# RunpeiDong/ACT

Hardware: AMD Instinct MI355X
Metric: stage2_pretrain_point_clouds_per_sec (higher is better)
Workload: dtype f32

## Files before the change

### act_amd/_abi.py

```python
import ctypes

_vp, _i, _f, _sz = ctypes.c_void_p, ctypes.c_int, ctypes.c_float, ctypes.c_size_t
_u, _u64, _ll, _str = ctypes.c_uint, ctypes.c_uint64, ctypes.c_longlong, ctypes.c_char_p
_d = ctypes.c_double
_P = ctypes.POINTER


class GemmEpilogue(ctypes.Structure):
    _fields_ = [("alpha", _f), ("act", _i), ("accumulate", _i), ("rows_per_scale", _i), ("ldr", _i), ("ldaux", _i),
                ("res_row_div", _i), ("bias", _vp), ("rowscale", _vp), ("res", _vp), ("aux", _vp)]


class GemmTnProblem(ctypes.Structure):
    _fields_ = [("A", _vp), ("lda", _i), ("B", _vp), ("ldb", _i), ("C", _vp), ("ldc", _i), ("M", _i), ("N", _i), ("bias_out", _vp)]


class GemmFx(ctypes.Structure):
    _fields_ = ([(n, _vp) for n in ("a_scale", "a_shift", "b_scale", "b_shift", "tile_stats", "gmax", "garg")] + [("group", _i), ("store_c", _i)]
                + [(n, _vp) for n in ("sa_src", "sa_arg", "ep_src", "ep_arg", "row_groups")])


class BlockParams(ctypes.Structure):
    _fields_ = [(n, _vp) for n in ("norm1_w", "norm1_b", "qkv_w", "qkv_b", "proj_w", "proj_b", "norm2_w", "norm2_b",
                                   "fc1_w", "fc1_b", "fc2_w", "fc2_b")]
# ... 92 lines not shown
    "act_bn_tiles_finalize_f32": [_vp, _i, _i, _i, _vp, _vp, _f, _f, _vp, _vp, _vp, _vp, _vp, _vp, _vp],
    "act_layernorm_fwd_f32": [_vp, _vp, _vp, _vp, _vp, _vp, _vp, _vp, _i, _i, _f, _vp],
    "act_prompt_layernorm_fwd_f32": [_vp, _vp, _i, _i, _i, _f, _u64, _vp, _vp, _vp, _f, _vp, _vp],
    "act_prompt_rows_fwd_f32": [_vp, _vp, _vp, _i, _i, _i, _f, _u64, _vp, _vp],
    "act_prompt_rows_bwd_f32": [_vp, _vp, _i, _i, _i, _f, _u64, _vp, _vp, _vp],
    "act_layernorm_bwd_workspace": (_sz, [_i, _i]),
    "act_layernorm_bwd_f32": [_vp, _vp, _vp, _vp, _vp, _vp, _vp, _vp, _vp, _i, _vp, _sz, _i, _i, _vp],
    "act_colsum_workspace": (_sz, [_i, _i]),
    "act_colsum_f32": [_vp, _i, _i, _i, _vp, _i, _vp, _sz, _vp],
    "act_attention_fwd_f32": [_vp, _vp, _vp, _i, _i, _i, _i, _f, _vp],
    "act_attention_fwd_prefix_f32": [_vp, _i, _vp, _i, _vp, _vp, _i, _i, _i, _f, _vp],
    "act_attention_bwd_f32": [_vp, _vp, _vp, _vp, _vp, _i, _i, _i, _i, _f, _vp],
    "act_attention_bwd_prefix_f32": [_vp, _i, _vp, _i, _vp, _vp, _vp, _vp, _vp, _i, _i, _i, _f, _vp],
    "act_cosine_loss_fwd_f32": [_vp, _vp, _i, _i, _f, _vp, _vp, _vp, _vp],
    "act_cosine_loss_bwd_f32": [_vp, _vp, _vp, _vp, _i, _i, _f, _vp, _vp],
    "act_regression_loss_fwd_f32": [_vp, _vp, _i, _i, _i, _vp, _vp, _vp],
    "act_regression_loss_bwd_f32": [_vp, _vp, _vp, _i, _i, _i, _vp, _vp],
    "act_softmax_xent_fwd_f32": [_vp, _vp, _i, _i, _vp, _vp, _vp, _vp],
    "act_softmax_xent_bwd_f32": [_vp, _vp, _vp, _vp, _i, _i, _vp, _vp],
    "act_colstats_workspace": (_sz, [_i, _i]),
    "act_bn_stats_f32": [_vp, _i, _i, _vp, _vp, _f, _f, _vp, _vp, _vp, _vp, _vp, _vp, _vp, _sz, _vp],
    "act_affine_act_f32": [_vp, _vp, _vp, _i, _i, _i, _vp, _vp],
    "act_bn_bwd_f32": [_vp, _vp, _vp, _vp, _vp, _vp, _i, _i, _i, _vp, _vp, _vp, _vp, _sz, _vp],
    "act_bn_bwd_groups_f32": [_vp, _vp, _vp, _vp, _vp, _vp, _i, _i, _i, _vp, _i, _vp, _vp, _vp, _vp, _sz, _vp],
    "act_col_mean_var_f32": [_vp, _i, _i, _vp, _vp, _vp, _sz, _vp],
    "act_bn_bwd_sums_f32": [_vp, _vp, _vp, _vp, _vp, _vp, _i, _i, _i, _vp, _vp, _vp, _sz, _vp],
    "act_bn_bwd_apply_f32": [_vp, _vp, _vp, _vp, _vp, _vp, _vp, _vp, _f, _i, _i, _i, _vp, _vp],
    "act_group_max_f32": [_vp, _i, _i, _i, _vp, _vp, _vp],
    "act_group_max_bwd_f32": [_vp, _vp, _i, _i, _i, _i, _vp, _vp],
    "act_group_max_bwd_matmul_f32": [_vp, _vp, _i, _i, _i, _vp, _i, _i, _vp, _i, _vp],
    "act_group_live_i32": [_vp, _i, _i, _vp, _vp],
    "act_group_max_bwd_matmul_live_f32": [_vp, _vp, _i, _i, _i, _vp, _i, _i, _vp, _i, _vp, _vp],
    "act_group_max_bwd_wgrad_workspace": (_sz, [_i, _i, _i, _i]),
    "act_group_max_bwd_wgrad_f32": [_vp, _vp, _i, _i, _i, _vp, _i, _i, _vp, _vp, _vp, _i, _vp, _sz, _vp],
    "act_group_sum_f32": [_vp, _i, _i, _i, _vp, _vp],
    "act_edge_gn_lrelu_max_f32": [_vp, _i, _i, _vp, _i, _i, _i, _i, _i, _vp, _vp, _f, _f, _vp, _vp, _i, _i, _vp],
    "act_edge_gn_lrelu_max_bwd_f32": [_vp, _i, _i, _vp, _i, _i, _i, _i, _i, _vp, _vp, _vp, _f, _vp, _i, _vp, _vp, _vp, _vp],
    "act_edge_bwd_lds": [_i],
    "act_gn_gumbel_argmax_gather_f32": [_vp, _i, _i, _i, _i, _vp, _vp, _f, _f, _vp, _u64, _vp, _f, _vp, _i, _vp, _vp, _vp, _vp, _vp],
    "act_gumbel_softmax_fwd_f32": [_vp, _i, _i, _vp, _u64, _f, _vp, _vp],
    "act_gumbel_softmax_bwd_f32": [_vp, _vp, _i, _i, _f, _vp, _vp],
    "act_kl_uniform_fwd_f32": [_vp, _i, _i, _i, _vp, _vp, _vp, _vp],
    "act_kl_uniform_bwd_f32": [_vp, _vp, _vp, _vp, _i, _i, _i, _vp, _vp],
    "act_split_bf16x2_f32": [_vp, _i, _i, _i, _vp, _vp, _vp],
    "act_sgemm_nt_bf16x3_supported": [_i, _i, _i],
    "act_sgemm_nt_bf16x3_f32": [_i, _i, _i, _vp, _vp, _vp, _vp, _vp, _i, _epi, _vp],
    "act_layernorm_fwd_planes_f32": [_vp, _vp, _vp, _vp, _vp, _vp, _vp, _vp, _vp, _vp, _i, _i, _f, _vp],
    "act_prompt_layernorm_fwd_planes_f32": [_vp, _vp, _i, _i, _i, _f, _u64, _vp, _vp, _vp, _f, _vp, _vp, _vp],
    "act_attention_fwd_prefix_planes_f32": [_vp, _i, _vp, _i, _vp, _vp, _vp, _vp, _i, _i, _i, _f, _vp],
    "act_sgemm_nt_bf16x3_planes_f32": [_i, _i, _i, _vp, _vp, _vp, _vp, _vp, _i, _vp, _vp, _epi, _vp],
    "act_split_f16x2_f32": [_vp, _i, _i, _i, _f, _vp, _vp, _vp, _vp],
    "act_sgemm_nt_f16x3_supported": [_i, _i, _i],
    "act_sgemm_nt_f16x3_planes_f32": [_i, _i, _i, _vp, _vp, _f, _vp, _vp, _vp, _vp, _i, _vp, _vp, _f, _epi, _vp],
    "act_layernorm_fwd_f16_planes_f32": [_vp, _vp, _vp, _vp, _vp, _vp, _vp, _vp, _f, _vp, _vp, _i, _i, _f, _vp],
    "act_attention_fwd_prefix_f16_planes_f32": [_vp, _i, _vp, _i, _vp, _vp, _vp, _f, _vp, _i, _i, _i, _f, _vp],
    "act_gemm_tune_set": [_i] * 7,
    "act_gemm_tune_get": [_i] * 5 + [_P(_i), _P(_i)],
    "act_gemm_tune_clear": [],
    "act_gemm_tile_info": [_i] + [_P(_i)] * 4,
    "act_scale_rows_f32": [_vp, _vp, _i, _i, _i, _vp, _vp],
    "act_bn_eval_affine_f32": [_vp, _vp, _vp, _vp, _f, _i, _vp, _vp, _vp],
    "act_composite_collect_begin": [],
    "act_composite_collect_end": [_P(_i), _i],
    "act_composite_shutdown": [],
    "act_block_saved_floats": (_sz, [_dims]),
    "act_block_fwd_f32": [_dims, _blk, _vp, _vp, _vp, _vp, _i, _vp, _vp, _vp, _sz, _vp],
    "act_block_bwd_scratch_floats": (_sz, [_dims]),
    "act_block_bwd_f32": [_dims, _blk, _vp, _vp, _vp, _vp, _vp, _blk, _vp, _vp, _sz, _vp, _sz, _vp, _vp],
    "act_block_stack_saved_floats": (_sz, [_dims, _i, _i]),
    "act_block_stack_bwd_scratch_floats": (_sz, [_dims, _i]),
    "act_block_stack_fwd_f32": [_dims, _P(BlockStack), _vp, _vp, _i, _vp, _vp, _vp, _sz, _vp],
    "act_block_stack_bwd_f32": [_dims, _P(BlockStack), _vp, _vp, _vp, _vp, _vp, _vp, _vp, _vp, _sz, _vp, _sz, _vp, _vp],
    "act_add_f32": [_vp, _vp, _vp, _ll, _vp],
    "act_prefix_block_saved_floats": (_sz, [_dims, _i]),
    "act_prefix_block_fwd_f32": [_dims, _i, _blk, _vp, _vp, _vp, _vp, _i, _vp, _vp, _vp, _sz, _vp],
    "act_prefix_block_fwd_kv_f32": [_dims, _i, _blk, _vp, _vp, _vp, _vp, _vp, _vp, _sz, _vp],
    "act_prompt_kv_sparse": [_i],
    "act_prompt_kv_workspace": (_sz, [_i, _i, _i, _i]),
    "act_prompt_kv_fwd_f32": [_vp, _vp, _i, _i, _i, _i, _f, _u64, _vp, _vp, _vp, _f, _vp, _vp, _vp, _vp, _sz, _vp, _sz, _vp],
    "act_prefix_block_bwd_scratch_floats": (_sz, [_dims, _i]),
    "act_prefix_block_bwd_f32": [_dims, _i, _blk, _vp, _vp, _vp, _vp, _vp, _vp, _vp, _sz, _vp],
    "act_prefix_vit_scratch_floats": (_sz, [_P(PrefixVit)]),
    "act_prefix_vit_fwd_bf16x3_f32": [_P(PrefixVit), _x3, _vp, _vp, _vp, _vp, _vp, _sz, _vp],
    "act_prefix_block_fwd_bf16x3_f32": [_dims, _i, _blk, _x3, _vp, _vp, _vp, _i, _vp, _vp, _vp, _sz, _vp],
    "act_prefix_block_bwd_bf16x3_f32": [_dims, _i, _blk, _x3, _vp, _vp, _vp, _vp, _vp, _vp, _vp, _sz, _vp],
    "act_prefix_vit_fwd_f32": [_P(PrefixVit), _vp, _vp, _vp, _vp, _vp, _sz, _vp],
    "act_prefix_vit_fwd_f16x3_f32": [_P(PrefixVit), _P(VitF16x3), _vp, _vp, _vp, _vp, _vp, _sz, _vp],
    "act_pointnet_saved_floats": (_sz, [_pnd]),
    "act_pointnet_fwd_f32": [_pnd, _pnp, _vp, _i, _i, _vp, _vp, _vp, _sz, _vp],
    "act_pointnet_fwd_groups_f32": [_pnd, _pnp, _vp, _i, _i, _vp, _vp, _vp, _i, _vp, _sz, _vp],
    "act_pointnet_bwd_scratch_floats": (_sz, [_pnd]),
    "act_pointnet_bwd_f32": [_pnd, _pnp, _vp, _vp, _vp, _P(PointnetGrads), _vp, _vp, _sz, _vp],
    "act_dgcnn_scratch_floats": (_sz, [_P(Dgcnn)]),
    "act_dgcnn_features_f32": [_P(Dgcnn), _vp, _vp, _vp, _vp, _vp, _sz, _vp],
    "act_dgcnn_features_f16x3_f32": [_P(Dgcnn), _P(DgcnnF16x3), _vp, _vp, _vp, _vp, _vp, _sz, _vp],
    "act_three_nn_f32": [_vp, _vp, _i, _i, _i, _vp, _vp, _vp, _vp, _vp],
    "act_interp_rows_fwd_f32": [_vp, _vp, _vp, _vp, _vp, _vp, _i, _i, _i, _i, _vp, _vp],
    "act_interp_rows_bwd_f32": [_vp, _vp, _vp, _vp, _i, _i, _i, _i, _vp, _vp],
    "act_interp_xyz_grad_workspace": (_sz, [_ll, _i]),
    "act_interp_xyz_grad_f32": [_vp, _vp, _ll, _i, _vp, _vp, _vp, _sz, _vp],
    "act_log_softmax_fwd_f32": [_vp, _ll, _i, _vp, _vp],
    "act_log_softmax_bwd_f32": [_vp, _vp, _ll, _i, _vp, _vp],
    "act_nll_weighted_workspace": (_sz, [_ll]),
    "act_nll_weighted_fwd_f32": [_vp, _vp, _vp, _ll, _i, _vp, _vp, _vp, _vp, _sz, _vp],
    "act_nll_weighted_bwd_f32": [_vp, _vp, _vp, _vp, _ll, _i, _vp, _vp],
    "act_confusion_i64": [_vp, _vp, _ll, _i, _vp, _vp],
# ... 65 lines not shown
```

### act_amd/csrc/gemm_bf16x3.hip

```cpp
#include "gemm_common.h"
#include "split_f16.h"
#include <stdlib.h>

typedef short bf16x8 __attribute__((ext_vector_type(8)));
typedef _Float16 f16x8 __attribute__((ext_vector_type(8)));
typedef unsigned u32x4v __attribute__((ext_vector_type(4)));

namespace {

__device__ __forceinline__ unsigned bf16_rne(float x) {
    unsigned u = __float_as_uint(x);
    u += 0x7FFFu + ((u >> 16) & 1u);
    return u >> 16;
}

__global__ __launch_bounds__(256) void split_bf16x2_kernel(const float* __restrict__ x, int K4, int ldx, long long n4, unsigned short* __restrict__ hi,
                                                           unsigned short* __restrict__ lo) {
    for (long long i = (long long)blockIdx.x * blockDim.x + threadIdx.x; i < n4; i += (long long)gridDim.x * blockDim.x) {
        const long long row = i / K4; const int c4 = (int)(i - row * K4);
        const float4 v = *reinterpret_cast<const float4*>(x + row * ldx + c4 * 4);
        const float e[4] = {v.x, v.y, v.z, v.w};
        unsigned h[4], l[4];
#pragma unroll
        for (int j = 0; j < 4; ++j) {
            h[j] = bf16_rne(e[j]);
            l[j] = bf16_rne(e[j] - __uint_as_float(h[j] << 16));
        }
        reinterpret_cast<uint2*>(hi)[i] = make_uint2(h[0] | (h[1] << 16), h[2] | (h[3] << 16));
        reinterpret_cast<uint2*>(lo)[i] = make_uint2(l[0] | (l[1] << 16), l[2] | (l[3] << 16));
    }
}
__global__ __launch_bounds__(256) void split_f16x2_kernel(const float* __restrict__ x, int K4, int ldx, long long n4, float scale,
                                                          const float* __restrict__ row_scale, unsigned short* __restrict__ h1, unsigned short* __restrict__ h2) {
    for (long long i = (long long)blockIdx.x * blockDim.x + threadIdx.x; i < n4; i += (long long)gridDim.x * blockDim.x) {
        const long long row = i / K4; const int c4 = (int)(i - row * K4);
        const float4 v = *reinterpret_cast<const float4*>(x + row * ldx + c4 * 4);
        store_f16_planes4(h1, h2, (size_t)i, v, row_scale ? scale * row_scale[row] : scale);
    }
}

constexpr int BK = 32;
constexpr int LROW = 40;

struct X3Params {
    const unsigned short *Ah, *Al, *Bh, *Bl;
    float* C; int ldc;
    unsigned short *Oh, *Ol;
    int M, N, K;
    act_gemm_epilogue_t epi;
    const float* b_inv; float a_inv, o_scale;
};

template <bool F16>
__device__ __forceinline__ f32x4 x3_mfma(const bf16x8& b, const bf16x8& a, const f32x4& c) {
    if constexpr (F16) return __builtin_amdgcn_mfma_f32_16x16x32_f16(__builtin_bit_cast(f16x8, b), __builtin_bit_cast(f16x8, a), c, 0, 0, 0);
    else return __builtin_amdgcn_mfma_f32_16x16x32_bf16(b, a, c, 0, 0, 0);
}

template <int BM, int BN, int ACT, bool PLANES, bool F16>
__global__ __launch_bounds__(256, 2) void sgemm_nt_bf16x3_kernel(const X3Params p) {
    constexpr int TM = BM / 32, TN = BN / 32;
    constexpr int PA = BM * LROW, PB = BN * LROW;
    constexpr int NA = BM / 64, NB = BN / 64;
    constexpr int STAGE = 2 * (PA + PB);
    __shared__ __attribute__((aligned(16))) unsigned short L[2 * STAGE];
    const int tid = threadIdx.x, lane = tid & 63, wave = tid >> 6;
    const int wm = wave >> 1, wn = wave & 1;
    const int tiles_n = p.N / BN, tiles_m = p.M / BM;
    int wg = blockIdx.x;
    {
        const int nwg = tiles_m * tiles_n, q = nwg >> 3, r = nwg & 7, xcd = wg & 7, loc = wg >> 3;
        wg = (xcd < r ? xcd * (q + 1) : r * (q + 1) + (xcd - r) * q) + loc;
    }
    constexpr int GM = 8;
    const int per_group = GM * tiles_n, group = wg / per_group, first_m = group * GM;
    const int gsz = min(tiles_m - first_m, GM), in_group = wg - group * per_group;
    const int tile_m = first_m + in_group % gsz, tile_n = in_group / gsz;
    const int m0 = tile_m * BM, n0 = tile_n * BN;
    const int K = p.K, ntiles = K / BK, last = ntiles - 1;

    constexpr int X = F16 ? 1 : 0;
    f32x4 acc[X + 1][TM][TN];
#pragma unroll
    for (int x = 0; x <= X; ++x)
#pragma unroll
        for (int i = 0; i < TM; ++i)
#pragma unroll
            for (int j = 0; j < TN; ++j) acc[x][i][j] = f32x4{0.f, 0.f, 0.f, 0.f};

    const int srow = tid >> 2, sch = tid & 3;
    const size_t goa = (size_t)(m0 + srow) * K + sch * 8, gob = (size_t)(n0 + srow) * K + sch * 8;
    const unsigned short* gA[2] = {p.Ah + goa, p.Al + goa};
    const unsigned short* gB[2] = {p.Bh + gob, p.Bl + gob};
    u32x4v ra0[2][NA], rb0[2][NB], ra1[2][NA], rb1[2][NB];
    const int s_off = srow * LROW + sch * 8;
    const int r = lane & 15, g = lane >> 4;
    const int a_off = (wm * (BM / 2) + r) * LROW + g * 8, b_off = (wn * (BN / 2) + r) * LROW + g * 8;
#define X3_LOAD(RA, RB, T)                                                                                                             \
    _Pragma("unroll") for (int s_ = 0; s_ < 2; ++s_) {                                                                                 \
        _Pragma("unroll") for (int i_ = 0; i_ < NA; ++i_) RA[s_][i_] = *reinterpret_cast<const u32x4v*>(gA[s_] + (size_t)(64 * i_) * K + (T) * BK); \
        _Pragma("unroll") for (int i_ = 0; i_ < NB; ++i_) RB[s_][i_] = *reinterpret_cast<const u32x4v*>(gB[s_] + (size_t)(64 * i_) * K + (T) * BK); \
    }
#define X3_STORE(RA, RB, STG)                                                                                                          \
    _Pragma("unroll") for (int s_ = 0; s_ < 2; ++s_) {                                                                                 \
        _Pragma("unroll") for (int i_ = 0; i_ < NA; ++i_) *reinterpret_cast<u32x4v*>(&L[(STG) * STAGE + s_ * PA + s_off + 64 * i_ * LROW]) = RA[s_][i_];           \
        _Pragma("unroll") for (int i_ = 0; i_ < NB; ++i_) *reinterpret_cast<u32x4v*>(&L[(STG) * STAGE + 2 * PA + s_ * PB + s_off + 64 * i_ * LROW]) = RB[s_][i_];  \
    }
#define X3_COMPUTE(STG)                                                                                                                \
    {                                                                                                                                  \
        const unsigned short* As_ = L + (STG) * STAGE; const unsigned short* Bs_ = As_ + 2 * PA;                                       \
        bf16x8 af[TM][2];                                                                                                              \
        _Pragma("unroll") for (int i_ = 0; i_ < TM; ++i_)                                                                              \
            _Pragma("unroll") for (int s_ = 0; s_ < 2; ++s_) af[i_][s_] = *reinterpret_cast<const bf16x8*>(&As_[s_ * PA + a_off + i_ * 16 * LROW]); \
        _Pragma("unroll") for (int j_ = 0; j_ < TN; ++j_) {                                                                            \
            bf16x8 bf[2];                                                                                                              \
            _Pragma("unroll") for (int s_ = 0; s_ < 2; ++s_) bf[s_] = *reinterpret_cast<const bf16x8*>(&Bs_[s_ * PB + b_off + j_ * 16 * LROW]); \
             \
             \
            _Pragma("unroll") for (int i_ = 0; i_ < TM; ++i_) acc[X][i_][j_] = x3_mfma<F16>(bf[0], af[i_][1], acc[X][i_][j_]);           \
            _Pragma("unroll") for (int i_ = 0; i_ < TM; ++i_) acc[X][i_][j_] = x3_mfma<F16>(bf[1], af[i_][0], acc[X][i_][j_]);           \
            _Pragma("unroll") for (int i_ = 0; i_ < TM; ++i_) acc[0][i_][j_] = x3_mfma<F16>(bf[0], af[i_][0], acc[0][i_][j_]);           \
        }                                                                                                                              \
    }
    X3_LOAD(ra0, rb0, 0)
    X3_LOAD(ra1, rb1, min(1, last))
    X3_STORE(ra0, rb0, 0)
    __syncthreads();
    for (int t = 0; t < ntiles; t += 2) {
        X3_LOAD(ra0, rb0, min(t + 2, last))
        X3_COMPUTE(0)
        X3_STORE(ra1, rb1, 1)
        __syncthreads();
        X3_LOAD(ra1, rb1, min(t + 3, last))
        X3_COMPUTE(1)
        X3_STORE(ra0, rb0, 0)
        __syncthreads();
    }
#undef X3_LOAD
#undef X3_STORE
#undef X3_COMPUTE
    const bool vec = (((uintptr_t)p.C | (uintptr_t)p.epi.bias | (uintptr_t)p.epi.res | (uintptr_t)p.epi.aux) & 15) == 0 &&
                     ((p.ldc | (p.epi.res ? p.epi.ldr : 0) | (p.epi.aux ? p.epi.ldaux : 0)) & 3) == 0;
#pragma unroll
    for (int i = 0; i < TM; ++i)
#pragma unroll
        for (int j = 0; j < TN; ++j) {
            const int row = m0 + wm * (BM / 2) + i * 16 + r;
            const int col = n0 + wn * (BN / 2) + j * 16 + g * 4;
            float4 v = make_float4(acc[0][i][j][0], acc[0][i][j][1], acc[0][i][j][2], acc[0][i][j][3]);
            if constexpr (F16) {
                const float4 bi = *reinterpret_cast<const float4*>(p.b_inv + col);
                constexpr float W = 1.0f / 2048.0f;
                v.x = __builtin_fmaf(acc[1][i][j][0], W, v.x) * bi.x * p.a_inv; v.y = __builtin_fmaf(acc[1][i][j][1], W, v.y) * bi.y * p.a_inv;
                v.z = __builtin_fmaf(acc[1][i][j][2], W, v.z) * bi.z * p.a_inv; v.w = __builtin_fmaf(acc[1][i][j][3], W, v.w) * bi.w * p.a_inv;
            }
            if (vec) v = epilogue_apply4_act<ACT>(p.epi, v, row, col);
            else {
                v.x = epilogue_apply<ACT>(p.epi, v.x, row, col); v.y = epilogue_apply<ACT>(p.epi, v.y, row, col + 1);
                v.z = epilogue_apply<ACT>(p.epi, v.z, row, col + 2); v.w = epilogue_apply<ACT>(p.epi, v.w, row, col + 3);
            }
            if (!PLANES || p.C) {
                float* cp = p.C + (size_t)row * p.ldc + col;
                if (vec) *reinterpret_cast<float4*>(cp) = v; else { cp[0] = v.x; cp[1] = v.y; cp[2] = v.z; cp[3] = v.w; }
            }
            if constexpr (PLANES && F16) {
                store_f16_planes4(p.Oh, p.Ol, ((size_t)row * p.N + col) >> 2, v, p.o_scale);
            } else if constexpr (PLANES) {
                const float e[4] = {v.x, v.y, v.z, v.w};
                unsigned h[4], l[4];
#pragma unroll
                for (int q = 0; q < 4; ++q) { h[q] = bf16_rne(e[q]); l[q] = bf16_rne(e[q] - __uint_as_float(h[q] << 16)); }
                const size_t o = (size_t)row * p.N + col;
                *reinterpret_cast<uint2*>(p.Oh + o) = make_uint2(h[0] | (h[1] << 16), h[2] | (h[3] << 16));
                *reinterpret_cast<uint2*>(p.Ol + o) = make_uint2(l[0] | (l[1] << 16), l[2] | (l[3] << 16));
            }
        }
}

template <int BM, int BN, bool F16>
int launch_x3(const X3Params& p, hipStream_t s) {
    const dim3 grid((p.M / BM) * (p.N / BN));
    const bool planes = p.Oh != nullptr;
    switch (p.epi.act) {
        case ACT_EPI_NONE:
            if (planes) hipLaunchKernelGGL((sgemm_nt_bf16x3_kernel<BM, BN, ACT_EPI_NONE, true, F16>), grid, dim3(256), 0, s, p);
            else        hipLaunchKernelGGL((sgemm_nt_bf16x3_kernel<BM, BN, ACT_EPI_NONE, false, F16>), grid, dim3(256), 0, s, p);
            break;
        case ACT_EPI_GELU:
            if (planes) hipLaunchKernelGGL((sgemm_nt_bf16x3_kernel<BM, BN, ACT_EPI_GELU, true, F16>), grid, dim3(256), 0, s, p);
            else        hipLaunchKernelGGL((sgemm_nt_bf16x3_kernel<BM, BN, ACT_EPI_GELU, false, F16>), grid, dim3(256), 0, s, p);
            break;
        case ACT_EPI_MUL_GELU_GRAD:
            if (planes) hipLaunchKernelGGL((sgemm_nt_bf16x3_kernel<BM, BN, ACT_EPI_MUL_GELU_GRAD, true, F16>), grid, dim3(256), 0, s, p);
            else        hipLaunchKernelGGL((sgemm_nt_bf16x3_kernel<BM, BN, ACT_EPI_MUL_GELU_GRAD, false, F16>), grid, dim3(256), 0, s, p);
            break;
        default: return ACT_E_BADARG;
    }
    ACT_LAUNCH_CHECK();
    return 0;
}

}

extern "C" int act_split_bf16x2_f32(const float* x, int R, int K, int ldx, uint16_t* hi, uint16_t* lo, act_stream_t stream) {
    if (!x || !hi || !lo) return ACT_E_NULLPTR;
    if (R < 0 || K <= 0 || (K & 3) || ldx < K || (ldx & 3) || (((uintptr_t)x | (uintptr_t)hi | (uintptr_t)lo) & 15)) return ACT_E_BADARG;
    const long long n4 = (long long)R * K / 4; if (n4 == 0) return 0;
    hipStream_t s = (hipStream_t)stream;
    ActProfScope ps(KID_ELTWISE, s, 0.0, 8.0 * R * (double)K);
    long long g = (n4 + 255) / 256; if (g > 8192) g = 8192;
    hipLaunchKernelGGL(split_bf16x2_kernel, dim3((unsigned)g), dim3(256), 0, s, x, K / 4, ldx, n4, hi, lo);
    ACT_LAUNCH_CHECK(); return 0;
}

extern "C" int act_sgemm_nt_bf16x3_supported(int M, int N, int K) { return M > 0 && N > 0 && K > 0 && M % 128 == 0 && N % 128 == 0 && K % 64 == 0; }

extern "C" int act_sgemm_nt_bf16x3_f32(int M, int N, int K, const uint16_t* a_hi, const uint16_t* a_lo, const uint16_t* b_hi, const uint16_t* b_lo,
                                       float* C, int ldc, const act_gemm_epilogue_t* epilogue, act_stream_t stream) {
    return act_sgemm_nt_bf16x3_planes_f32(M, N, K, a_hi, a_lo, b_hi, b_lo, C, ldc, nullptr, nullptr, epilogue, stream);
}

extern "C" int act_sgemm_nt_bf16x3_planes_f32(int M, int N, int K, const uint16_t* a_hi, const uint16_t* a_lo, const uint16_t* b_hi, const uint16_t* b_lo,
                                              float* C, int ldc, uint16_t* out_hi, uint16_t* out_lo, const act_gemm_epilogue_t* epilogue,
                                              act_stream_t stream) {
    if (!a_hi || !a_lo || !b_hi || !b_lo || (!C && !out_hi) || ((out_hi == nullptr) != (out_lo == nullptr))) return ACT_E_NULLPTR;
    if (!act_sgemm_nt_bf16x3_supported(M, N, K) || (C && ldc < N)) return ACT_E_BADARG;
    if ((((uintptr_t)a_hi | (uintptr_t)a_lo | (uintptr_t)b_hi | (uintptr_t)b_lo | (uintptr_t)out_hi | (uintptr_t)out_lo) & 15)) return ACT_E_BADARG;
    X3Params p{};
    p.Ah = a_hi; p.Al = a_lo; p.Bh = b_hi; p.Bl = b_lo; p.C = C; p.ldc = ldc; p.M = M; p.N = N; p.K = K; p.Oh = out_hi; p.Ol = out_lo;
    if (epilogue) p.epi = *epilogue; else { p.epi = act_gemm_epilogue_t{}; p.epi.alpha = 1.0f; }
    if (p.epi.accumulate || (p.epi.act != ACT_EPI_NONE && p.epi.act != ACT_EPI_GELU && p.epi.act != ACT_EPI_MUL_GELU_GRAD)) return ACT_E_BADARG;
    hipStream_t s = (hipStream_t)stream;
    ActProfScope ps(KID_GEMM_BF16X3, s, 2.0 * M * (double)N * K, 4.0 * ((double)M * K + (double)N * K + (double)M * N));
    return launch_x3<128, 128, false>(p, s);
}

extern "C" int act_split_f16x2_f32(const float* x, int R, int K, int ldx, float scale, const float* row_scale, uint16_t* h1, uint16_t* h2,
                                   act_stream_t stream) {
    if (!x || !h1 || !h2) return ACT_E_NULLPTR;
    if (R < 0 || K <= 0 || (K & 3) || ldx < K || (ldx & 3) || !(scale > 0.f) || (((uintptr_t)x | (uintptr_t)h1 | (uintptr_t)h2) & 15)) return ACT_E_BADARG;
    const long long n4 = (long long)R * K / 4; if (n4 == 0) return 0;
    hipStream_t s = (hipStream_t)stream;
    ActProfScope ps(KID_ELTWISE, s, 0.0, 8.0 * R * (double)K);
    long long g = (n4 + 255) / 256; if (g > 8192) g = 8192;
    hipLaunchKernelGGL(split_f16x2_kernel, dim3((unsigned)g), dim3(256), 0, s, x, K / 4, ldx, n4, scale, row_scale, h1, h2);
    ACT_LAUNCH_CHECK(); return 0;
}

extern "C" int act_sgemm_nt_f16x3_supported(int M, int N, int K) { return act_sgemm_nt_bf16x3_supported(M, N, K); }

extern "C" int act_sgemm_nt_f16x3_planes_f32(int M, int N, int K, const uint16_t* a_h1, const uint16_t* a_h2, float a_scale, const uint16_t* b_h1,
                                             const uint16_t* b_h2, const float* b_inv_scale, float* C, int ldc, uint16_t* out_h1, uint16_t* out_h2,
                                             float out_scale, const act_gemm_epilogue_t* epilogue, act_stream_t stream) {
    if (!a_h1 || !a_h2 || !b_h1 || !b_h2 || !b_inv_scale || (!C && !out_h1) || ((out_h1 == nullptr) != (out_h2 == nullptr))) return ACT_E_NULLPTR;
    if (!act_sgemm_nt_f16x3_supported(M, N, K) || (C && ldc < N) || !(a_scale > 0.f) || (out_h1 && !(out_scale > 0.f))) return ACT_E_BADARG;
    if ((((uintptr_t)a_h1 | (uintptr_t)a_h2 | (uintptr_t)b_h1 | (uintptr_t)b_h2 | (uintptr_t)out_h1 | (uintptr_t)out_h2 | (uintptr_t)b_inv_scale) & 15))
        return ACT_E_BADARG;
    X3Params p{};
    p.Ah = a_h1; p.Al = a_h2; p.Bh = b_h1; p.Bl = b_h2; p.C = C; p.ldc = ldc; p.M = M; p.N = N; p.K = K; p.Oh = out_h1; p.Ol = out_h2;
    p.b_inv = b_inv_scale; p.a_inv = 1.0f / a_scale; p.o_scale = out_scale;
    if (epilogue) p.epi = *epilogue; else { p.epi = act_gemm_epilogue_t{}; p.epi.alpha = 1.0f; }
    if (p.epi.accumulate || (p.epi.act != ACT_EPI_NONE && p.epi.act != ACT_EPI_GELU && p.epi.act != ACT_EPI_MUL_GELU_GRAD)) return ACT_E_BADARG;
    hipStream_t s = (hipStream_t)stream;
    ActProfScope ps(KID_GEMM_BF16X3, s, 2.0 * M * (double)N * K, 4.0 * ((double)M * K + (double)N * K + (double)M * N));
    return launch_x3<128, 128, true>(p, s);
}
```

### act_amd/kernels.py

```python
import ctypes
import os

import numpy as np

import torch

from . import _C
from ._abi import GemmEpilogue, GemmTnProblem

EPI_NONE, EPI_GELU, EPI_RELU, EPI_MUL_GELU_GRAD, EPI_MUL_RELU_MASK = 0, 1, 2, 3, 4

lib, ptr, stream, check = _C.lib, _C.ptr, _C.stream, _C.check

_WS = {}
_WS_BYTES = 160 << 20


def workspace(device, nbytes=_WS_BYTES, stream_handle=None):
    idx = device.index if device.index is not None else torch.cuda.current_device()
    key = (idx, _C.stream_handle(idx) if stream_handle is None else stream_handle)
    w = _WS.get(key)
    if w is None or w.numel() * 4 < nbytes:
        w = torch.empty(max(nbytes, _WS_BYTES) // 4, dtype=torch.float32, device=device)
        _WS[key] = w
# ... 127 lines not shown
                                           None, None, T, D, float(eps), stream()), "act_layernorm_fwd_planes_f32")
    return planes


def gemm_nt_bf16x3(a_planes, b_planes, bias=None, act=EPI_NONE, res=None, out=None, planes_out=None):
    _, M, Kd = a_planes.shape
    _, N, Kb = b_planes.shape
    if Kd != Kb or a_planes.dtype != torch.bfloat16 or b_planes.dtype != torch.bfloat16 or not (a_planes.is_contiguous() and b_planes.is_contiguous()):
        raise _C.ActHipError("gemm_nt_bf16x3: contiguous bf16 planes [2, rows, K] with equal K expected")
    if not lib.act_sgemm_nt_bf16x3_supported(M, N, Kd):
        raise _C.ActHipError(f"gemm_nt_bf16x3: unsupported shape {M} x {N} x {Kd} (M, N % 128, K % 64)")
    if out is None:
        out = torch.empty(M, N, dtype=torch.float32, device=a_planes.device)
    e = GemmEpilogue(alpha=1.0, act=act, accumulate=0, rows_per_scale=0, ldr=(res.stride(0) if res is not None else 0), ldaux=0, res_row_div=0,
                     bias=ptr(bias), rowscale=None, res=ptr(res), aux=None)
    if planes_out is not None:
        if planes_out.dtype != torch.bfloat16 or tuple(planes_out.shape) != (2, M, N) or not planes_out.is_contiguous():
            raise _C.ActHipError("gemm_nt_bf16x3: planes_out must be a contiguous bf16 tensor [2, M, N]")
        check(lib.act_sgemm_nt_bf16x3_planes_f32(M, N, Kd, ptr(a_planes[0]), ptr(a_planes[1]), ptr(b_planes[0]), ptr(b_planes[1]), ptr(out), out.stride(0),
                                                 ptr(planes_out[0]), ptr(planes_out[1]), ctypes.byref(e), stream()), "act_sgemm_nt_bf16x3_planes_f32")
        return out
    check(lib.act_sgemm_nt_bf16x3_f32(M, N, Kd, ptr(a_planes[0]), ptr(a_planes[1]), ptr(b_planes[0]), ptr(b_planes[1]), ptr(out), out.stride(0),
                                      ctypes.byref(e), stream()), "act_sgemm_nt_bf16x3_f32")
    return out


def f16x3_row_scales(w):
    mx = w.detach().abs().amax(dim=1).float()
    e = torch.frexp(mx).exponent
    e = torch.where(mx > 0, e, torch.full_like(e, 15))
    one = torch.ones(e.shape, dtype=torch.float32, device=w.device)
    return torch.ldexp(one, 15 - e), torch.ldexp(one, e - 15)


def split_f16x2(x, scale=1.0, row_scale=None, out=None):
    x = _f32rows(x, "x")
    R, Kd = x.shape
    if out is None:
        out = torch.empty(2, R, Kd, dtype=torch.float16, device=x.device)
    check(lib.act_split_f16x2_f32(_C.ptr_rows(x), R, Kd, x.stride(0), float(scale), ptr(_f32c(row_scale)) if row_scale is not None else None,
                                  ptr(out[0]), ptr(out[1]), stream()), "act_split_f16x2_f32")
    return out


def layernorm_f16_planes(x, gamma, beta, eps, scale, pos=None):
    x = _f32c(x)
    T, D = x.shape
    planes = torch.empty(2, T, D, dtype=torch.float16, device=x.device)
    check(lib.act_layernorm_fwd_f16_planes_f32(ptr(x), ptr(_f32c(pos)) if pos is not None else None, ptr(gamma), ptr(beta), None, None, ptr(planes[0]),
                                               ptr(planes[1]), float(scale), None, None, T, D, float(eps), stream()), "act_layernorm_fwd_f16_planes_f32")
    return planes


def gemm_nt_f16x3(a_planes, a_scale, b_planes, b_inv_scale, bias=None, act=EPI_NONE, res=None, out=None, planes_out=None, out_scale=1.0):
    _, M, Kd = a_planes.shape
    _, N, Kb = b_planes.shape
    if Kd != Kb or a_planes.dtype != torch.float16 or b_planes.dtype != torch.float16 or not (a_planes.is_contiguous() and b_planes.is_contiguous()):
        raise _C.ActHipError("gemm_nt_f16x3: contiguous f16 planes [2, rows, K] with equal K expected")
    if not lib.act_sgemm_nt_f16x3_supported(M, N, Kd):
        raise _C.ActHipError(f"gemm_nt_f16x3: unsupported shape {M} x {N} x {Kd} (M, N % 128, K % 64)")
    b_inv_scale = _f32c(b_inv_scale)
    if b_inv_scale.numel() != N:
        raise _C.ActHipError("gemm_nt_f16x3: b_inv_scale must hold one value per row of b")
    if out is None:
        out = torch.empty(M, N, dtype=torch.float32, device=a_planes.device)
    e = GemmEpilogue(alpha=1.0, act=act, accumulate=0, rows_per_scale=0, ldr=(res.stride(0) if res is not None else 0), ldaux=0, res_row_div=0,
                     bias=ptr(bias), rowscale=None, res=ptr(res), aux=None)
    oh, ol = (None, None)
    if planes_out is not None:
        if planes_out.dtype != torch.float16 or tuple(planes_out.shape) != (2, M, N) or not planes_out.is_contiguous():
            raise _C.ActHipError("gemm_nt_f16x3: planes_out must be a contiguous f16 tensor [2, M, N]")
        oh, ol = ptr(planes_out[0]), ptr(planes_out[1])
    check(lib.act_sgemm_nt_f16x3_planes_f32(M, N, Kd, ptr(a_planes[0]), ptr(a_planes[1]), float(a_scale), ptr(b_planes[0]), ptr(b_planes[1]), ptr(b_inv_scale),
                                            ptr(out), out.stride(0), oh, ol, float(out_scale), ctypes.byref(e), stream()), "act_sgemm_nt_f16x3_planes_f32")
    return out


_GEMM_CACHE = {}
AUTOTUNE = os.environ.get("ACT_GEMM_AUTOTUNE", "1") != "0"
AUTOTUNE_FULL = os.environ.get("ACT_GEMM_AUTOTUNE", "1") == "full"
_TUNE_FILE = os.environ.get("ACT_GEMM_TUNE_FILE") or os.path.join(os.path.dirname(os.path.abspath(__file__)), "gemm_tune_gfx950.json")
_GEMM_TABLE = {}
_MAX_SPLIT = int(os.environ.get("ACT_GEMM_MAX_SPLIT", "0"))
if os.environ.get("ACT_GEMM_TUNE_TABLE", "1") != "0" and os.path.exists(_TUNE_FILE):
    import json as _json
    with open(_TUNE_FILE) as _fh:
        _GEMM_TABLE = {tuple(int(v) for v in k.split(",")): tuple(c) for k, c in _json.load(_fh)["configs"].items()}
    if _MAX_SPLIT > 0:
        _GEMM_TABLE = {k: c for k, c in _GEMM_TABLE.items() if c[1] <= _MAX_SPLIT or k[4] > 8192}
_NEW_TUNED = {}
if os.environ.get("ACT_GEMM_TUNE_SAVE"):
    import atexit as _atexit

    def _dump_tuned(path=os.environ["ACT_GEMM_TUNE_SAVE"].replace("%p", str(os.getpid()))):
        import json
        merged = dict(_GEMM_TABLE); merged.update(_NEW_TUNED)
        with open(path, "w") as f:
            json.dump({"arch": "gfx950", "key": "a_kmajor,b_kmajor,M,N,K", "value": "[tile id, split-K]",
                       "configs": {",".join(str(v) for v in k): list(c) for k, c in sorted(merged.items())}}, f, indent=0)
    _atexit.register(_dump_tuned)


def stable_split(M, N, K, ws_bytes):
    nb = -(-M // 64) * -(-N // 64)
    if nb >= 384 or K < 1024:
        return 1
    s = max(1, min(8, K // 256, int(round(512.0 / nb))))
    while s > 1 and s * M * N * 4 > ws_bytes:
        s -= 1
    return s


_TILE_BN = {}


def tile_bn(tile):
    if not _TILE_BN:
        bn = ctypes.c_int()
        for t in range(1, 64):
            if lib.act_gemm_tile_info(t, None, ctypes.byref(bn), None, None) == 0:
                _TILE_BN[t] = bn.value
    return _TILE_BN[tile]


def stable_candidates(a, b, ak, bk, M, N, K, ws):
    aligned = ((a.data_ptr() | b.data_ptr()) & 15) == 0 and a.stride(0) % 4 == 0 and b.stride(0) % 4 == 0
    if not aligned or K % 32 != 0:
# ... 2039 lines not shown
```

### include/act_hip.h

```cpp
#ifndef ACT_HIP_H
#define ACT_HIP_H
#include <stdint.h>
#include <stddef.h>
#ifdef __cplusplus
extern "C" {
#endif

typedef void* act_stream_t;

#define ACT_E_BADARG   (-1)
#define ACT_E_NULLPTR  (-2)
#define ACT_E_UNSUPPORTED (-3)

int         act_version(void);
const char* act_arch(void);

int         act_prof_enable(int on);
int         act_prof_reset(void);
int         act_prof_num_kernels(void);
const char* act_prof_kernel_name(int id);
int         act_prof_read(int id, double* total_ms, long long* launches, double* flops, double* bytes);

size_t act_fps_scratch_floats(int B, int N);
int act_fps_f32(const float* xyz, int B, int N, int G, int32_t* idx_out, float* centers_out,
// ... 150 lines not shown
int act_bn_bwd_apply_f32(const float* x, const float* dy, const float* scale, const float* shift, const float* mean, const float* rstd,
                         const float* sum_dy, const float* sum_dy_xhat, float count, int relu, int R, int C, float* dx, act_stream_t stream);
int act_group_max_f32(const float* in, int G, int n, int C, float* out, int32_t* arg, act_stream_t stream);
int act_group_max_bwd_f32(const float* dout, const int32_t* arg, int G, int n, int C, int accumulate, float* din,
                          act_stream_t stream);
int act_group_max_bwd_matmul_f32(const float* dout, const int32_t* arg, int G, int n, int C, const float* w, int ldw, int N, float* dx, int lddx,
                                 act_stream_t stream);
int act_group_live_i32(const float* d, int G, int C, int32_t* live, act_stream_t stream);
int act_group_max_bwd_matmul_live_f32(const float* dout, const int32_t* arg, int G, int n, int C, const float* w, int ldw, int N, float* dx, int lddx,
                                      const int32_t* live, act_stream_t stream);
size_t act_group_max_bwd_wgrad_workspace(int G, int n, int C, int N);
int act_group_max_bwd_wgrad_f32(const float* dout, const int32_t* arg, int G, int n, int C, const float* x, int ldx, int N, const float* scale,
                                const float* shift, float* dw, int lddw, float* workspace, size_t workspace_bytes, act_stream_t stream);
int act_group_sum_f32(const float* in, int G, int n, int C, float* out, act_stream_t stream);

int act_edge_gn_lrelu_max_f32(const float* yz, int ldy, int zoff, const int64_t* idx, int B, int G, int k, int C,
                              int groups, const float* gamma, const float* beta, float eps, float slope, float* stats,
                              float* out, int ldo, int ooff, act_stream_t stream);
int act_edge_gn_lrelu_max_bwd_f32(const float* yz, int ldy, int zoff, const int64_t* idx, int B, int G, int k, int C, int groups,
                                  const float* gamma, const float* beta, const float* stats, float slope,
                                  const float* dout, int ldd, float* dyz, float* part, float* mstat, act_stream_t stream);
int act_edge_bwd_lds(int on);
int act_gn_gumbel_argmax_gather_f32(const float* h, int B, int G, int C, int groups, const float* gamma, const float* beta,
                                    float eps, float slope, const float* noise, uint64_t seed, const uint64_t* seed_dev, float tau,
                                    const float* codebook, int D, float* stats, int64_t* index_out, float* out,
                                    float* logits_out, act_stream_t stream);
int act_gumbel_softmax_fwd_f32(const float* logits, int R, int C, const float* noise, uint64_t seed, float tau, float* y,
                               act_stream_t stream);
int act_gumbel_softmax_bwd_f32(const float* y, const float* dy, int R, int C, float tau, float* dlogits, act_stream_t stream);
int act_kl_uniform_fwd_f32(const float* logits, int B, int G, int C, float* lse, float* qbar, float* klv_out, act_stream_t stream);
int act_kl_uniform_bwd_f32(const float* logits, const float* lse, const float* qbar, const float* grad_klv, int B, int G, int C,
                           float* dlogits, act_stream_t stream);

int act_split_bf16x2_f32(const float* x, int R, int K, int ldx, uint16_t* hi, uint16_t* lo, act_stream_t stream);
int act_sgemm_nt_bf16x3_supported(int M, int N, int K);
int act_sgemm_nt_bf16x3_f32(int M, int N, int K, const uint16_t* a_hi, const uint16_t* a_lo, const uint16_t* b_hi, const uint16_t* b_lo,
                            float* C, int ldc, const act_gemm_epilogue_t* epilogue, act_stream_t stream);
int act_layernorm_fwd_planes_f32(const float* x, const float* pos, const float* gamma, const float* beta, float* xin_out, float* y,
                                 uint16_t* y_hi, uint16_t* y_lo, float* mean , float* rstd , int T, int D, float eps,
                                 act_stream_t stream);
int act_prompt_layernorm_fwd_planes_f32(const float* tok, const float* ppos, int B, int P, int D, float drop_p, uint64_t seed,
                                        const uint64_t* seed_dev, const float* gamma, const float* beta, float eps, uint16_t* y_hi, uint16_t* y_lo,
                                        act_stream_t stream);
int act_attention_fwd_prefix_planes_f32(const float* kv0, int S0, const float* qkv1, int Sq, float* out, uint16_t* out_hi, uint16_t* out_lo, float* lse,
                                        int B, int H, int head_dim, float scale, act_stream_t stream);
int act_sgemm_nt_bf16x3_planes_f32(int M, int N, int K, const uint16_t* a_hi, const uint16_t* a_lo, const uint16_t* b_hi, const uint16_t* b_lo,
                                   float* C, int ldc, uint16_t* out_hi, uint16_t* out_lo, const act_gemm_epilogue_t* epilogue, act_stream_t stream);

int act_split_f16x2_f32(const float* x, int R, int K, int ldx, float scale, const float* row_scale, uint16_t* h1, uint16_t* h2, act_stream_t stream);
int act_sgemm_nt_f16x3_supported(int M, int N, int K);
int act_sgemm_nt_f16x3_planes_f32(int M, int N, int K, const uint16_t* a_h1, const uint16_t* a_h2, float a_scale, const uint16_t* b_h1,
                                  const uint16_t* b_h2, const float* b_inv_scale, float* C, int ldc, uint16_t* out_h1, uint16_t* out_h2, float out_scale,
                                  const act_gemm_epilogue_t* epilogue, act_stream_t stream);
int act_layernorm_fwd_f16_planes_f32(const float* x, const float* pos, const float* gamma, const float* beta, float* xin_out, float* y,
                                     uint16_t* y_h1, uint16_t* y_h2, float plane_scale, float* mean , float* rstd , int T, int D,
                                     float eps, act_stream_t stream);
int act_attention_fwd_prefix_f16_planes_f32(const float* kv0, int S0, const float* qkv1, int Sq, float* out, uint16_t* out_h1, uint16_t* out_h2,
                                            float plane_scale, float* lse, int B, int H, int head_dim, float scale, act_stream_t stream);

int act_gemm_tune_set(int a_kmajor, int b_kmajor, int M, int N, int K, int tile, int splits);
int act_gemm_tune_get(int a_kmajor, int b_kmajor, int M, int N, int K, int* tile, int* splits);
int act_gemm_tune_clear(void);
#define ACT_GEMM_LAYOUT_TN 1
#define ACT_GEMM_LAYOUT_TT 2
#define ACT_GEMM_LAYOUT_NN 4
#define ACT_GEMM_LAYOUT_NT 8
#define ACT_GEMM_NEED_ANY           0
#define ACT_GEMM_NEED_FULL_OR_MTAIL 1
#define ACT_GEMM_NEED_FULL          2
#define ACT_GEMM_NEED_OFFSET32      4
int act_gemm_tile_info(int tile, int* bm, int* bn, int* layouts, int* need);

int act_scale_rows_f32(const float* x, const float* gate, int T, int D, int rows_per_scale, float* y, act_stream_t stream);
int act_bn_eval_affine_f32(const float* gamma, const float* beta, const float* running_mean, const float* running_var, float eps,
                           int C, float* scale, float* shift, act_stream_t stream);

int act_composite_collect_begin(void);
int act_composite_collect_end(int* shapes, int max);
int act_composite_shutdown(void);

typedef struct {
    const float *norm1_w, *norm1_b, *qkv_w, *qkv_b , *proj_w, *proj_b, *norm2_w, *norm2_b,
                *fc1_w, *fc1_b, *fc2_w, *fc2_b;
} act_block_params_t;
typedef struct {
    float *norm1_w, *norm1_b, *qkv_w, *qkv_b , *proj_w, *proj_b, *norm2_w, *norm2_b, *fc1_w, *fc1_b, *fc2_w, *fc2_b;
} act_block_grads_t;
typedef struct { int B, S, D, heads, hidden; float eps; } act_block_dims_t;

size_t act_block_saved_floats(const act_block_dims_t* d);
int act_block_fwd_f32(const act_block_dims_t* d, const act_block_params_t* w, const float* x, const float* pos,
                      const float* gate1, const float* gate2, int keep_for_backward, float* saved, float* out,
                      float* workspace, size_t workspace_bytes, act_stream_t stream);
size_t act_block_bwd_scratch_floats(const act_block_dims_t* d);
int act_block_bwd_f32(const act_block_dims_t* d, const act_block_params_t* w, const float* gate1, const float* gate2,
                      const float* saved, const float* dout, float* dx, const act_block_grads_t* grads, float* scratch,
                      float* workspace, size_t workspace_bytes, float* side_workspace, size_t side_workspace_bytes,
                      act_stream_t stream, act_stream_t side_stream);

typedef struct {
    int depth;
    const act_block_params_t* blocks;
    const float* const* gate1;
    const float* const* gate2;
} act_block_stack_t;
size_t act_block_stack_saved_floats(const act_block_dims_t* d, int depth, int keep_for_backward);
// ... 240 lines not shown
```

Baseline: 6922.

## Add 128x192 eight-wave tile to f16x3 GEMM with wave-quantization tile picker

Generalizes the split-precision MFMA GEMM kernel over the number of waves per workgroup and adds a 128x192 tile that runs 8 waves, including partial-row staging for tiles whose height is not a multiple of the rows loaded per pass. A heuristic picks 192 over 128 when N is divisible by 384 and the estimated count of waves of workgroups across the CUs is lower, to reduce tail under-utilization. The larger tile uses one workgroup per CU with more LDS and registers, which could lower occupancy or latency hiding. An environment variable forces the old tile.

```diff
diff --git a/act_amd/_abi.py b/act_amd/_abi.py
--- a/act_amd/_abi.py
+++ b/act_amd/_abi.py
@@ -168,6 +168,8 @@
     "act_split_f16x2_f32": [_vp, _i, _i, _i, _f, _vp, _vp, _vp, _vp],
     "act_sgemm_nt_f16x3_supported": [_i, _i, _i],
     "act_sgemm_nt_f16x3_planes_f32": [_i, _i, _i, _vp, _vp, _f, _vp, _vp, _vp, _vp, _i, _vp, _vp, _f, _epi, _vp],
+    "act_sgemm_nt_f16x3_pick_tile": [_i, _i, _i, _i],
+    "act_sgemm_nt_f16x3_planes_tile_f32": [_i, _i, _i, _vp, _vp, _f, _vp, _vp, _vp, _vp, _i, _vp, _vp, _f, _epi, _vp, _i],
     "act_layernorm_fwd_f16_planes_f32": [_vp, _vp, _vp, _vp, _vp, _vp, _vp, _vp, _f, _vp, _vp, _i, _i, _f, _vp],
     "act_attention_fwd_prefix_f16_planes_f32": [_vp, _i, _vp, _i, _vp, _vp, _vp, _f, _vp, _i, _i, _i, _f, _vp],
     "act_gemm_tune_set": [_i] * 7,
diff --git a/act_amd/csrc/gemm_bf16x3.hip b/act_amd/csrc/gemm_bf16x3.hip
--- a/act_amd/csrc/gemm_bf16x3.hip
+++ b/act_amd/csrc/gemm_bf16x3.hip
@@ -57,15 +57,20 @@
     else return __builtin_amdgcn_mfma_f32_16x16x32_bf16(b, a, c, 0, 0, 0);
 }
 
-template <int BM, int BN, int ACT, bool PLANES, bool F16>
-__global__ __launch_bounds__(256, 2) void sgemm_nt_bf16x3_kernel(const X3Params p) {
-    constexpr int TM = BM / 32, TN = BN / 32;
+constexpr int x3_wgs_per_cu(int waves) { return waves <= 4 ? 2 : 1; }
+
+template <int BM, int BN, int WGM, int WGN, int ACT, bool PLANES, bool F16>
+__global__ __launch_bounds__(64 * WGM * WGN, x3_wgs_per_cu(WGM * WGN) * WGM * WGN / 4) void sgemm_nt_bf16x3_kernel(const X3Params p) {
+    constexpr int NT = 64 * WGM * WGN, RP = NT / 4;
+    constexpr int WM = BM / WGM, WN = BN / WGN;
+    constexpr int TM = WM / 16, TN = WN / 16;
     constexpr int PA = BM * LROW, PB = BN * LROW;
-    constexpr int NA = BM / 64, NB = BN / 64;
+    constexpr int NA = (BM + RP - 1) / RP, NB = (BN + RP - 1) / RP;
     constexpr int STAGE = 2 * (PA + PB);
+    static_assert(WM % 16 == 0 && WN % 16 == 0 && BM % 16 == 0 && BN % 16 == 0, "whole 16 x 16 blocks per wave, whole waves per staging row test");
     __shared__ __attribute__((aligned(16))) unsigned short L[2 * STAGE];
     const int tid = threadIdx.x, lane = tid & 63, wave = tid >> 6;
-    const int wm = wave >> 1, wn = wave & 1;
+    const int wm = wave / WGN, wn = wave % WGN;
     const int tiles_n = p.N / BN, tiles_m = p.M / BM;
     int wg = blockIdx.x;
     {
@@ -95,16 +100,24 @@
     u32x4v ra0[2][NA], rb0[2][NB], ra1[2][NA], rb1[2][NB];
     const int s_off = srow * LROW + sch * 8;
     const int r = lane & 15, g = lane >> 4;
-    const int a_off = (wm * (BM / 2) + r) * LROW + g * 8, b_off = (wn * (BN / 2) + r) * LROW + g * 8;
+    const int a_off = (wm * WM + r) * LROW + g * 8, b_off = (wn * WN + r) * LROW + g * 8;
+    const long long ta = (long long)(min(srow + RP * (NA - 1), BM - 1) - srow) * K, tb = (long long)(min(srow + RP * (NB - 1), BN - 1) - srow) * K;
+#define X3_WHOLE(I, ROWS) (RP * ((I) + 1) <= (ROWS))
 #define X3_LOAD(RA, RB, T)                                                                                                             \
     _Pragma("unroll") for (int s_ = 0; s_ < 2; ++s_) {                                                                                 \
-        _Pragma("unroll") for (int i_ = 0; i_ < NA; ++i_) RA[s_][i_] = *reinterpret_cast<const u32x4v*>(gA[s_] + (size_t)(64 * i_) * K + (T) * BK); \
-        _Pragma("unroll") for (int i_ = 0; i_ < NB; ++i_) RB[s_][i_] = *reinterpret_cast<const u32x4v*>(gB[s_] + (size_t)(64 * i_) * K + (T) * BK); \
+        _Pragma("unroll") for (int i_ = 0; i_ < NA; ++i_)                                                                              \
+            RA[s_][i_] = *reinterpret_cast<const u32x4v*>(gA[s_] + (X3_WHOLE(i_, BM) ? (long long)(RP * i_) * K : ta) + (T) * BK);      \
+        _Pragma("unroll") for (int i_ = 0; i_ < NB; ++i_)                                                                              \
+            RB[s_][i_] = *reinterpret_cast<const u32x4v*>(gB[s_] + (X3_WHOLE(i_, BN) ? (long long)(RP * i_) * K : tb) + (T) * BK);      \
     }
 #define X3_STORE(RA, RB, STG)                                                                                                          \
     _Pragma("unroll") for (int s_ = 0; s_ < 2; ++s_) {                                                                                 \
-        _Pragma("unroll") for (int i_ = 0; i_ < NA; ++i_) *reinterpret_cast<u32x4v*>(&L[(STG) * STAGE + s_ * PA + s_off + 64 * i_ * LROW]) = RA[s_][i_];           \
-        _Pragma("unroll") for (int i_ = 0; i_ < NB; ++i_) *reinterpret_cast<u32x4v*>(&L[(STG) * STAGE + 2 * PA + s_ * PB + s_off + 64 * i_ * LROW]) = RB[s_][i_];  \
+        _Pragma("unroll") for (int i_ = 0; i_ < NA; ++i_)                                                                              \
+            if (X3_WHOLE(i_, BM) || srow + RP * i_ < BM)                                                                               \
+                *reinterpret_cast<u32x4v*>(&L[(STG) * STAGE + s_ * PA + s_off + RP * i_ * LROW]) = RA[s_][i_];                         \
+        _Pragma("unroll") for (int i_ = 0; i_ < NB; ++i_)                                                                              \
+            if (X3_WHOLE(i_, BN) || srow + RP * i_ < BN)                                                                               \
+                *reinterpret_cast<u32x4v*>(&L[(STG) * STAGE + 2 * PA + s_ * PB + s_off + RP * i_ * LROW]) = RB[s_][i_];                \
     }
 #define X3_COMPUTE(STG)                                                                                                                \
     {                                                                                                                                  \
@@ -136,6 +149,7 @@
         X3_STORE(ra0, rb0, 0)
         __syncthreads();
     }
+#undef X3_WHOLE
 #undef X3_LOAD
 #undef X3_STORE
 #undef X3_COMPUTE
@@ -145,8 +159,8 @@
     for (int i = 0; i < TM; ++i)
 #pragma unroll
         for (int j = 0; j < TN; ++j) {
-            const int row = m0 + wm * (BM / 2) + i * 16 + r;
-            const int col = n0 + wn * (BN / 2) + j * 16 + g * 4;
+            const int row = m0 + wm * WM + i * 16 + r;
+            const int col = n0 + wn * WN + j * 16 + g * 4;
             float4 v = make_float4(acc[0][i][j][0], acc[0][i][j][1], acc[0][i][j][2], acc[0][i][j][3]);
             if constexpr (F16) {
                 const float4 bi = *reinterpret_cast<const float4*>(p.b_inv + col);
@@ -177,22 +191,22 @@
         }
 }
 
-template <int BM, int BN, bool F16>
+template <int BM, int BN, int WGM, int WGN, bool F16>
 int launch_x3(const X3Params& p, hipStream_t s) {
-    const dim3 grid((p.M / BM) * (p.N / BN));
+    const dim3 grid((p.M / BM) * (p.N / BN)), block(64 * WGM * WGN);
     const bool planes = p.Oh != nullptr;
     switch (p.epi.act) {
         case ACT_EPI_NONE:
-            if (planes) hipLaunchKernelGGL((sgemm_nt_bf16x3_kernel<BM, BN, ACT_EPI_NONE, true, F16>), grid, dim3(256), 0, s, p);
-            else        hipLaunchKernelGGL((sgemm_nt_bf16x3_kernel<BM, BN, ACT_EPI_NONE, false, F16>), grid, dim3(256), 0, s, p);
+            if (planes) hipLaunchKernelGGL((sgemm_nt_bf16x3_kernel<BM, BN, WGM, WGN, ACT_EPI_NONE, true, F16>), grid, block, 0, s, p);
+            else        hipLaunchKernelGGL((sgemm_nt_bf16x3_kernel<BM, BN, WGM, WGN, ACT_EPI_NONE, false, F16>), grid, block, 0, s, p);
             break;
         case ACT_EPI_GELU:
-            if (planes) hipLaunchKernelGGL((sgemm_nt_bf16x3_kernel<BM, BN, ACT_EPI_GELU, true, F16>), grid, dim3(256), 0, s, p);
-            else        hipLaunchKernelGGL((sgemm_nt_bf16x3_kernel<BM, BN, ACT_EPI_GELU, false, F16>), grid, dim3(256), 0, s, p);
+            if (planes) hipLaunchKernelGGL((sgemm_nt_bf16x3_kernel<BM, BN, WGM, WGN, ACT_EPI_GELU, true, F16>), grid, block, 0, s, p);
+            else        hipLaunchKernelGGL((sgemm_nt_bf16x3_kernel<BM, BN, WGM, WGN, ACT_EPI_GELU, false, F16>), grid, block, 0, s, p);
             break;
         case ACT_EPI_MUL_GELU_GRAD:
-            if (planes) hipLaunchKernelGGL((sgemm_nt_bf16x3_kernel<BM, BN, ACT_EPI_MUL_GELU_GRAD, true, F16>), grid, dim3(256), 0, s, p);
-            else        hipLaunchKernelGGL((sgemm_nt_bf16x3_kernel<BM, BN, ACT_EPI_MUL_GELU_GRAD, false, F16>), grid, dim3(256), 0, s, p);
+            if (planes) hipLaunchKernelGGL((sgemm_nt_bf16x3_kernel<BM, BN, WGM, WGN, ACT_EPI_MUL_GELU_GRAD, true, F16>), grid, block, 0, s, p);
+            else        hipLaunchKernelGGL((sgemm_nt_bf16x3_kernel<BM, BN, WGM, WGN, ACT_EPI_MUL_GELU_GRAD, false, F16>), grid, block, 0, s, p);
             break;
         default: return ACT_E_BADARG;
     }
@@ -232,7 +246,7 @@
     if (p.epi.accumulate || (p.epi.act != ACT_EPI_NONE && p.epi.act != ACT_EPI_GELU && p.epi.act != ACT_EPI_MUL_GELU_GRAD)) return ACT_E_BADARG;
     hipStream_t s = (hipStream_t)stream;
     ActProfScope ps(KID_GEMM_BF16X3, s, 2.0 * M * (double)N * K, 4.0 * ((double)M * K + (double)N * K + (double)M * N));
-    return launch_x3<128, 128, false>(p, s);
+    return launch_x3<128, 128, 2, 2, false>(p, s);
 }
 
 extern "C" int act_split_f16x2_f32(const float* x, int R, int K, int ldx, float scale, const float* row_scale, uint16_t* h1, uint16_t* h2,
@@ -249,13 +263,45 @@
 
 extern "C" int act_sgemm_nt_f16x3_supported(int M, int N, int K) { return act_sgemm_nt_bf16x3_supported(M, N, K); }
 
+extern "C" int act_sgemm_nt_f16x3_pick_tile(int M, int N, int K, int cus) {
+    if (!act_sgemm_nt_f16x3_supported(M, N, K) || cus <= 0) return 0;
+    if (N % 384) return 128;
+    const long long t128 = (long long)(M / 128) * (N / 128), t192 = (long long)(M / 128) * (N / 192);
+    const long long tail = t128 % (2 * cus);
+    const long long c128 = t128 / (2 * cus) * 4 + (tail == 0 ? 0 : tail <= cus ? 2 : 4), c192 = (t192 + cus - 1) / cus * 3;
+    return 8 * c192 <= 7 * c128 ? 192 : 128;
+}
+
+namespace {
+int x3_cu_count() {
+    static const int n = [] {
+        int dev = 0, v = 0;
+        if (hipGetDevice(&dev) != hipSuccess || hipDeviceGetAttribute(&v, hipDeviceAttributeMultiprocessorCount, dev) != hipSuccess || v <= 0) v = 256;
+        return v;
+    }();
+    return n;
+}
+bool x3_only_128() {
+    static const bool v = [] { const char* e = getenv("ACT_X3_TILE"); return e && atoi(e) == 128; }();
+    return v;
+}
+}
+
 extern "C" int act_sgemm_nt_f16x3_planes_f32(int M, int N, int K, const uint16_t* a_h1, const uint16_t* a_h2, float a_scale, const uint16_t* b_h1,
                                              const uint16_t* b_h2, const float* b_inv_scale, float* C, int ldc, uint16_t* out_h1, uint16_t* out_h2,
                                              float out_scale, const act_gemm_epilogue_t* epilogue, act_stream_t stream) {
+    return act_sgemm_nt_f16x3_planes_tile_f32(M, N, K, a_h1, a_h2, a_scale, b_h1, b_h2, b_inv_scale, C, ldc, out_h1, out_h2, out_scale, epilogue, stream, 0);
+}
+
+extern "C" int act_sgemm_nt_f16x3_planes_tile_f32(int M, int N, int K, const uint16_t* a_h1, const uint16_t* a_h2, float a_scale, const uint16_t* b_h1,
+                                                  const uint16_t* b_h2, const float* b_inv_scale, float* C, int ldc, uint16_t* out_h1, uint16_t* out_h2,
+                                                  float out_scale, const act_gemm_epilogue_t* epilogue, act_stream_t stream, int tile) {
     if (!a_h1 || !a_h2 || !b_h1 || !b_h2 || !b_inv_scale || (!C && !out_h1) || ((out_h1 == nullptr) != (out_h2 == nullptr))) return ACT_E_NULLPTR;
     if (!act_sgemm_nt_f16x3_supported(M, N, K) || (C && ldc < N) || !(a_scale > 0.f) || (out_h1 && !(out_scale > 0.f))) return ACT_E_BADARG;
     if ((((uintptr_t)a_h1 | (uintptr_t)a_h2 | (uintptr_t)b_h1 | (uintptr_t)b_h2 | (uintptr_t)out_h1 | (uintptr_t)out_h2 | (uintptr_t)b_inv_scale) & 15))
         return ACT_E_BADARG;
+    if (tile != 0 && tile != 128 && !(tile == 192 && N % 192 == 0)) return ACT_E_BADARG;
+    if (tile == 0) tile = x3_only_128() ? 128 : act_sgemm_nt_f16x3_pick_tile(M, N, K, x3_cu_count());
     X3Params p{};
     p.Ah = a_h1; p.Al = a_h2; p.Bh = b_h1; p.Bl = b_h2; p.C = C; p.ldc = ldc; p.M = M; p.N = N; p.K = K; p.Oh = out_h1; p.Ol = out_h2;
     p.b_inv = b_inv_scale; p.a_inv = 1.0f / a_scale; p.o_scale = out_scale;
@@ -263,5 +309,5 @@
     if (p.epi.accumulate || (p.epi.act != ACT_EPI_NONE && p.epi.act != ACT_EPI_GELU && p.epi.act != ACT_EPI_MUL_GELU_GRAD)) return ACT_E_BADARG;
     hipStream_t s = (hipStream_t)stream;
     ActProfScope ps(KID_GEMM_BF16X3, s, 2.0 * M * (double)N * K, 4.0 * ((double)M * K + (double)N * K + (double)M * N));
-    return launch_x3<128, 128, true>(p, s);
-}
+    return tile == 192 ? launch_x3<128, 192, 2, 4, true>(p, s) : launch_x3<128, 128, 2, 2, true>(p, s);
+}
diff --git a/act_amd/kernels.py b/act_amd/kernels.py
--- a/act_amd/kernels.py
+++ b/act_amd/kernels.py
@@ -203,7 +203,7 @@
     return planes
 
 
-def gemm_nt_f16x3(a_planes, a_scale, b_planes, b_inv_scale, bias=None, act=EPI_NONE, res=None, out=None, planes_out=None, out_scale=1.0):
+def gemm_nt_f16x3(a_planes, a_scale, b_planes, b_inv_scale, bias=None, act=EPI_NONE, res=None, out=None, planes_out=None, out_scale=1.0, tile=0):
     _, M, Kd = a_planes.shape
     _, N, Kb = b_planes.shape
     if Kd != Kb or a_planes.dtype != torch.float16 or b_planes.dtype != torch.float16 or not (a_planes.is_contiguous() and b_planes.is_contiguous()):
@@ -222,8 +222,9 @@
         if planes_out.dtype != torch.float16 or tuple(planes_out.shape) != (2, M, N) or not planes_out.is_contiguous():
             raise _C.ActHipError("gemm_nt_f16x3: planes_out must be a contiguous f16 tensor [2, M, N]")
         oh, ol = ptr(planes_out[0]), ptr(planes_out[1])
-    check(lib.act_sgemm_nt_f16x3_planes_f32(M, N, Kd, ptr(a_planes[0]), ptr(a_planes[1]), float(a_scale), ptr(b_planes[0]), ptr(b_planes[1]), ptr(b_inv_scale),
-                                            ptr(out), out.stride(0), oh, ol, float(out_scale), ctypes.byref(e), stream()), "act_sgemm_nt_f16x3_planes_f32")
+    check(lib.act_sgemm_nt_f16x3_planes_tile_f32(M, N, Kd, ptr(a_planes[0]), ptr(a_planes[1]), float(a_scale), ptr(b_planes[0]), ptr(b_planes[1]),
+                                                 ptr(b_inv_scale), ptr(out), out.stride(0), oh, ol, float(out_scale), ctypes.byref(e), stream(), int(tile)),
+          "act_sgemm_nt_f16x3_planes_tile_f32")
     return out
 
 
diff --git a/include/act_hip.h b/include/act_hip.h
--- a/include/act_hip.h
+++ b/include/act_hip.h
@@ -226,6 +226,10 @@
 int act_sgemm_nt_f16x3_planes_f32(int M, int N, int K, const uint16_t* a_h1, const uint16_t* a_h2, float a_scale, const uint16_t* b_h1,
                                   const uint16_t* b_h2, const float* b_inv_scale, float* C, int ldc, uint16_t* out_h1, uint16_t* out_h2, float out_scale,
                                   const act_gemm_epilogue_t* epilogue, act_stream_t stream);
+int act_sgemm_nt_f16x3_pick_tile(int M, int N, int K, int cus);
+int act_sgemm_nt_f16x3_planes_tile_f32(int M, int N, int K, const uint16_t* a_h1, const uint16_t* a_h2, float a_scale, const uint16_t* b_h1,
+                                       const uint16_t* b_h2, const float* b_inv_scale, float* C, int ldc, uint16_t* out_h1, uint16_t* out_h2,
+                                       float out_scale, const act_gemm_epilogue_t* epilogue, act_stream_t stream, int tile);
 int act_layernorm_fwd_f16_planes_f32(const float* x, const float* pos, const float* gamma, const float* beta, float* xin_out, float* y,
                                      uint16_t* y_h1, uint16_t* y_h2, float plane_scale, float* mean , float* rstd , int T, int D,
                                      float eps, act_stream_t stream);
```

New measurement: 7074 (median of 6 runs). +2.2%, better.
